# glennhickey/teHmm

Measured on NVIDIA B200. Metric: hmm_trellis_cells_per_sec_fwd_bwd_viterbi, higher is better.
Workload: dtype f32

## Files before the change

### tehmm_b200/csrc/api.cu

```cuda
#include "common.cuh"
#include <algorithm>
#include <cstdarg>
#include <cstdio>
#include <cstring>
#include <string>
#include <vector>

void tehmm_launch_strict_emission(cudaStream_t, const void *, int, int64_t, int, const double *, int, int, double *, double, const double *, unsigned long long *);
void tehmm_launch_strict_forward(cudaStream_t, int64_t, int, const double *, const double *, const double *, const double *, double *);
void tehmm_launch_strict_backward(cudaStream_t, int64_t, int, const double *, const double *, const double *, double *);
void tehmm_launch_strict_viterbi(cudaStream_t, int64_t, int, const double *, const double *, const double *, const double *, int16_t *, int64_t *, double *);
void tehmm_launch_strict_lneta(cudaStream_t, int64_t, int, const double *, const double *, const double *, const double *, double, const double *, double *);
void tehmm_launch_strict_accumulate(cudaStream_t, const void *, int, int64_t, int, double *, int, int, const double *, const double *);
void tehmm_launch_strict_counts(cudaStream_t, const void *, int, int, int64_t, int64_t, int, double *, int, int, const double *);
size_t tehmm_emission_table_budget(int K);
int tehmm_launch_emission(cudaStream_t, const TehmmModelDev &, const TehmmBatchDev &, int, const double *, void *, void *, double *, double *, int *, int, cudaError_t *, int64_t, int64_t);
bool tehmm_emission_rows_ok(const TehmmModelDev &, int, const double *);
cudaError_t tehmm_launch_forward(cudaStream_t, const TehmmModelDev &, const TehmmBatchDev &, int, const void *, const double *, const double *, void *, void *, void *, double *, const int *, int, int);
cudaError_t tehmm_launch_verify(cudaStream_t, const TehmmBatchDev &, int, int, void *, const void *, double, int, int, int *, int *, double *);
cudaError_t tehmm_launch_forward_logprob(cudaStream_t, const TehmmBatchDev &, int, int, const void *, const double *, const double *, double *);
cudaError_t tehmm_launch_backward(cudaStream_t, const TehmmModelDev &, const TehmmBatchDev &, int, int, const void *, const void *, const double *, void *, uint8_t *, double *, void *, void *, void *, void *, void *, const int *, int, int);
cudaError_t tehmm_launch_trans_reduce(cudaStream_t, const TehmmModelDev &, const TehmmBatchDev &, int, const void *, const void *, const void *, double *);
cudaError_t tehmm_launch_map_reduce(cudaStream_t, const TehmmBatchDev &, const double *, double *);
cudaError_t tehmm_launch_viterbi(cudaStream_t, const TehmmModelDev &, const TehmmBatchDev &, int, const void *, const double *, void *, void *, void *, const int *, int, int, const double *, double *);
bool tehmm_viterbi_dp_scores(const TehmmModelDev &, int, const double *);
cudaError_t tehmm_launch_vit_score_reduce(cudaStream_t, const TehmmBatchDev &, const double *, double *);
cudaError_t tehmm_launch_traceback(cudaStream_t, const TehmmModelDev &, const TehmmBatchDev &, int, const void *, const double *, uint8_t *, int64_t *, uint8_t *, uint8_t *, const uint8_t *, const int *, int, int);
cudaError_t tehmm_launch_tb_verify(cudaStream_t, const TehmmBatchDev &, uint8_t *, const uint8_t *, uint8_t *, int *, int *);
cudaError_t tehmm_launch_rescore(cudaStream_t, const TehmmModelDev &, const TehmmBatchDev &, const uint8_t *, const double *, const double *, double *, double *, int64_t, int64_t);
cudaError_t tehmm_launch_emission_stats(cudaStream_t, const TehmmModelDev &, const TehmmBatchDev &, int, const void *, const double *, double *, double *, int, int);
size_t tehmm_stats_smem_bytes(int tab_rows, int N, int K, int prec);
cudaError_t tehmm_launch_widen(cudaStream_t, const uint8_t *, int64_t *, int64_t);
cudaError_t tehmm_launch_forward_tile(cudaStream_t, const TehmmModelDev &, const TehmmBatchDev &, const float *, const double *, float *, float *, float *, double *, const int *, int, int, int64_t);
cudaError_t tehmm_launch_backward_tile(cudaStream_t, const TehmmModelDev &, const TehmmBatchDev &, int, const float *, const float *, float *, uint8_t *, double *, float *, float *, const int *, int, int, int64_t, int);
int tehmm_tile_warps(void);
bool tehmm_forward_umma_ok(const TehmmModelDev &, const TehmmBatchDev &, int, int64_t);
cudaError_t tehmm_launch_forward_umma(cudaStream_t, const TehmmModelDev &, const TehmmBatchDev &, const float *, const double *, float *, float *, float *, double *, int, int64_t, int *, int);
bool tehmm_backward_umma_ok(const TehmmModelDev &, const TehmmBatchDev &, int, int, int64_t);
cudaError_t tehmm_launch_backward_umma(cudaStream_t, const TehmmModelDev &, const TehmmBatchDev &, int, const float *, const float *, float *, uint8_t *, double *, float *, float *, int, int64_t, int *);
cudaError_t tehmm_launch_xi_tile(cudaStream_t, const TehmmModelDev &, const TehmmBatchDev &, const float *, const float *, double *, float *, double *, int);
size_t tehmm_xi_tile_scratch_bytes(int sms);
cudaError_t tehmm_launch_convert(cudaStream_t, int, const void *, double *, int64_t);
cudaError_t tehmm_launch_transfer_ops(cudaStream_t, const TehmmModelDev &, const TehmmChunk *, const int64_t *, int64_t, int, int, const void *, void *, double *, int);
cudaError_t tehmm_launch_ratio_fold(cudaStream_t, const TehmmModelDev &, int64_t, int, const double *, void *, double *, int);
cudaError_t tehmm_launch_ratio_diag(cudaStream_t, const TehmmModelDev &, const TehmmBatchDev &, int, const double *, const void *, double *, double *, int);
cudaError_t tehmm_launch_chain(cudaStream_t, const TehmmModelDev &, int, int, int, const int64_t *, const int64_t *, int64_t, const void *, const double *, const void *, void *);

static thread_local std::string g_err;
static int fail(int code, const char *fmt, ...)
{
    char buf[512];
    va_list ap;
    va_start(ap, fmt);
    vsnprintf(buf, sizeof buf, fmt, ap);
    va_end(ap);
    g_err = buf;
    return code;
}
void tehmm_set_error(int code, const char *msg) { (void)code; g_err = msg ? msg : ""; }
void tehmm_hostpipe_release(tehmm_ctx *c);
#define CU(x)                                                                                 \
    do {                                                                                      \
        cudaError_t e__ = (x);                                                                \
        if (e__ != cudaSuccess)                                                               \
            return fail(TEHMM_ECUDA, "%s failed: %s (%s:%d)", #x, cudaGetErrorString(e__),    \
                        __FILE__, __LINE__);                                                  \
    } while (0)

struct DevBuf {
    void *p = nullptr;
    ~DevBuf() { if (p) cudaFree(p); }
    cudaError_t alloc(size_t n) { return cudaMalloc(&p, n ? n : 1); }
    template <typename T> T *as() { return (T *)p; }
};

#define TEHMM_TRING 32
#define TEHMM_NPENDING 64
enum { TK_EMISSION, TK_FORWARD, TK_BACKWARD, TK_VITERBI_DP, TK_TRACEBACK, TK_RESCORE, TK_STATS, TK_XI, TEHMM_NTIMED };
static const char *const tk_names[TEHMM_NTIMED] = {"us_emission", "us_forward", "us_backward", "us_viterbi_dp",
                                                    "us_traceback", "us_rescore", "us_emission_stats", "us_xi"};

struct tehmm_ctx {
    int device = 0;
    int sms = 148;
    cudaStream_t stream = nullptr;
    cudaStream_t own_stream = nullptr;
    int64_t launches = 0;
    int64_t opt_chunk_tiles = 0, opt_warmup = 0, opt_max_repair = 0;
    int64_t opt_tile = 1, opt_fine_len = 0;
    int64_t opt_timing = 0;
    int64_t opt_umma = 0;
    int64_t opt_umma64 = 1;
    int *d_fault = nullptr;
    int64_t stat_umma_passes = 0;
    int64_t opt_rescore = 0;
    int64_t opt_bwd_tmap = 0;
    int64_t opt_xi_tile = 1;
    int64_t opt_fallback_after = 2;
    int64_t stat_fallbacks = 0, stat_fallback_chunks = 0, stat_noise_accepted = 0;
    double mix_rho = -1.0;
    std::vector<double> mix_A;
    int mix_N = 0;
    cudaEvent_t ev[TEHMM_NTIMED][TEHMM_TRING][2] = {};
    int ev_n[TEHMM_NTIMED] = {};
    int64_t stat_repair_fwd = 0, stat_repair_bwd = 0, stat_repair_vit = 0;
    int64_t stat_tile_passes = 0;
    int64_t stat_bad_fwd = 0, stat_bad_bwd = 0, stat_bad_vit = 0, stat_bad_tb = 0, stat_repair_tb = 0;
    int *h_nbad = nullptr;
    int64_t opt_defer = 0;
    int *h_pending = nullptr;
    int npending = 0;
    int64_t stat_deferred_checks = 0, stat_deferred_bad = 0;
    bool has_model = false;
    TehmmModelDev m{};
    void *model_blob = nullptr;
    size_t model_blob_bytes = 0;
    std::vector<unsigned char> model_key;
    bool has_batch = false;
    TehmmBatchDev b{};
    TehmmBatchDev bf{};
    std::vector<int64_t> batch_key;
    void *batch_blob = nullptr;
    size_t batch_blob_bytes = 0;
    int *d_seq_flag = nullptr;
    int64_t seq_flag_n = 0;
    int64_t max_tiles_per_chunk = 1;
    int64_t fine_len = 0;
};

// ... 56 lines not shown
{
    if (!c) return fail(TEHMM_EINVAL, "ctx is NULL");
    CU(cudaSetDevice(c->device));
    CU(cudaStreamSynchronize(c->stream));
    return TEHMM_OK;
}

int tehmm_ctx_set_stream(tehmm_ctx *c, uint64_t stream)
{
    if (!c) return fail(TEHMM_EINVAL, "ctx is NULL");
    CU(cudaSetDevice(c->device));
    CU(cudaStreamSynchronize(c->stream));
    c->stream = stream == UINT64_MAX ? c->own_stream : (cudaStream_t)(uintptr_t)stream;
    return TEHMM_OK;
}

uint64_t tehmm_ctx_stream(tehmm_ctx *c) { return c ? (uint64_t)(uintptr_t)c->stream : 0; }
int64_t tehmm_ctx_launch_count(tehmm_ctx *c) { return c ? c->launches : 0; }

int tehmm_ctx_set_option(tehmm_ctx *c, const char *name, int64_t v)
{
    if (!c || !name) return fail(TEHMM_EINVAL, "NULL argument");
    if (!strcmp(name, "chunk_tiles")) c->opt_chunk_tiles = v;
    else if (!strcmp(name, "warmup")) c->opt_warmup = v;
    else if (!strcmp(name, "max_repair")) c->opt_max_repair = v;
    else if (!strcmp(name, "tile")) c->opt_tile = v;
    else if (!strcmp(name, "timing")) { c->opt_timing = v; for (int i = 0; i < TEHMM_NTIMED; ++i) c->ev_n[i] = 0; }
    else if (!strcmp(name, "fine_len")) c->opt_fine_len = v;
    else if (!strcmp(name, "umma")) c->opt_umma = v;
    else if (!strcmp(name, "umma64")) c->opt_umma64 = v;
    else if (!strcmp(name, "xi_tile")) c->opt_xi_tile = v;
    else if (!strcmp(name, "defer")) c->opt_defer = v;
    else if (!strcmp(name, "bwd_tmap")) c->opt_bwd_tmap = v;
    else if (!strcmp(name, "rescore")) c->opt_rescore = v;
    else if (!strcmp(name, "fallback_after")) c->opt_fallback_after = v;
    else return fail(TEHMM_EINVAL, "unknown option %s", name);
    return TEHMM_OK;
}

static double mix_rho_of(tehmm_ctx *c)
{
    if (c->mix_rho >= 0.0) return c->mix_rho;
    const int N = c->mix_N;
    if (N <= 0 || c->mix_A.size() != (size_t)N * N) return 0.0;
    const std::vector<double> &A = c->mix_A;
    std::vector<double> pi(N, 1.0 / N), tmp(N), B((size_t)N * N), B2((size_t)N * N);
    for (int it = 0; it < 2000; ++it) {
        double sum = 0.0;
        for (int j = 0; j < N; ++j) tmp[j] = 0.0;
        for (int i = 0; i < N; ++i) {
            const double p = pi[i];
            for (int j = 0; j < N; ++j) tmp[j] += p * A[(size_t)i * N + j];
        }
        for (int j = 0; j < N; ++j) sum += tmp[j];
        for (int j = 0; j < N; ++j) pi[j] = sum > 0.0 ? tmp[j] / sum : 1.0 / N;
    }
    for (int i = 0; i < N; ++i) for (int j = 0; j < N; ++j) B[(size_t)i * N + j] = A[(size_t)i * N + j] - pi[j];
    double lognorm = 0.0;
    for (int sq = 0; sq < 8; ++sq) {
        double f = 0.0;
        for (double v : B) f += v * v;
        f = sqrt(f);
        if (!(f > 0.0)) { lognorm = -INFINITY; break; }
        for (double &v : B) v /= f;
        lognorm = 2.0 * (lognorm + log(f));
        for (int i = 0; i < N; ++i)
// ... 881 lines not shown
                       const double *d_ratios, void *d_post, uint8_t *d_map_states,
                       double *d_map_score, double *d_start_trans, void *d_scratch)
{
    RUN_PROLOGUE();
    if (!d_blin || !d_alpha || !d_scratch) return fail(TEHMM_EINVAL, "NULL argument");
    if ((flags & TEHMM_BWD_POSTERIORS) && !d_post) return fail(TEHMM_EINVAL, "POSTERIORS needs d_post");
    if ((flags & TEHMM_BWD_MAP) && (!d_map_states || !d_map_score)) return fail(TEHMM_EINVAL, "MAP needs d_map_states and d_map_score");
    if ((flags & TEHMM_BWD_TRANS) && !d_start_trans) return fail(TEHMM_EINVAL, "TRANS needs d_start_trans");
    const Scratch s = carve(c, prec);
    char *w = (char *)d_scratch;
    void *sv = w + s.start_vec, *ev = w + s.end_vec;
    double *mp = (double *)(w + s.part_a);
    int *bad = (int *)(w + s.bad), *nbad = (int *)(w + s.nbad);
    void *xi = w + s.xi, *xd = w + s.xdiag, *g0 = w + s.gamma0;
    const int grid = scan_grid(c);
    const bool xi_tile = use_tile(c, prec, d_ratios) && (flags & TEHMM_BWD_TRANS) && (flags & TEHMM_BWD_POSTERIORS) &&
                         !(flags & TEHMM_BWD_RENORM_EPS) && c->opt_xi_tile != 0;
    if (xi_tile) flags &= ~TEHMM_BWD_TRANS;
    const bool tile = use_tile(c, prec, d_ratios) && !(flags & TEHMM_BWD_TRANS);
    const bool wide_umma = c->opt_umma64 != 0 && c->opt_tile != 0 && prec == TEHMM_F32 && c->m.NS == 2 && c->m.LD == 64 &&
                           d_ratios == nullptr && c->b.nseq == 1 && !(flags & TEHMM_BWD_TRANS);
    const TehmmBatchDev &PB = (tile || wide_umma) ? c->bf : c->b;
    bool umma_used = false;
    auto launch = [&](int mode) -> cudaError_t {
        if (wide_umma && tehmm_backward_umma_ok(c->m, PB, flags, mode, c->fine_len)) {
            cudaError_t eu = tehmm_launch_backward_umma(st, c->m, PB, flags, (const float *)d_blin, (const float *)d_alpha, (float *)d_post,
                                                        d_map_states, mp, (float *)sv, (float *)ev, c->sms, c->fine_len, c->d_fault);
            if (eu == cudaSuccess) { c->stat_umma_passes += 1; umma_used = true; return eu; }
            if (eu != cudaErrorNotSupported) return eu;
            cudaGetLastError();
        }
        if (tile) {
            c->stat_tile_passes += 1;
            return tehmm_launch_backward_tile(st, c->m, PB, flags, (const float *)d_blin, (const float *)d_alpha, (float *)d_post, d_map_states, mp, (float *)sv, (float *)ev, bad, mode, c->sms, c->fine_len, (int)c->opt_bwd_tmap);
        }
        return tehmm_launch_backward(st, c->m, PB, prec, flags, d_blin, d_alpha, d_ratios, d_post, d_map_states, mp, xi, xd, g0, sv, ev, bad, mode, grid);
    };
    tk_begin(c, TK_BACKWARD);
    CU(launch(0));
    tk_end(c, TK_BACKWARD);
    c->launches += 1;
    double tol = tolerance(prec, false);
    const int64_t max_pass = c->opt_max_repair > 0 ? c->opt_max_repair : PB.nchunks + 1;
    int fb_rounds = 0;
    for (int64_t pass = 0;; ++pass) {
        CU(tehmm_launch_verify(st, PB, prec, c->m.NP, sv, ev, tol, -1, 1, bad, nbad, nullptr));
        c->launches += 1;
        int nb = 0;
        if (umma_used && pass == 0) CU(cudaMemcpyAsync(c->h_nbad + 1, c->d_fault, sizeof(int), cudaMemcpyDeviceToHost, st));
        if (read_nbad(c, nbad, &nb, !umma_used)) return TEHMM_ECUDA;
        if (umma_used && pass == 0 && c->h_nbad[1]) {
            CU(cudaMemsetAsync(c->d_fault, 0, sizeof(int), st));
            return fail(TEHMM_ECUDA, "bwd_umma_kernel: a barrier wait timed out (tensor-memory protocol fault)");
        }
        if (pass == 0) adapt_warmup(c, nb, PB.nchunks);
        if (nb == 0) break;
        if (pass >= max_pass) return fail(TEHMM_ESTATE, "backward repair did not converge (%d chunks left)", nb);
        if (c->opt_fallback_after >= 0 && pass >= c->opt_fallback_after && d_ratios == nullptr && fb_rounds < TEHMM_MAX_FALLBACK_ROUNDS) {
            if (resolve_flagged(c, st, PB, prec, 1, d_blin, sv, ev, bad, (int64_t)8 << (2 * fb_rounds))) return TEHMM_ECUDA;
            tol = tolerance_after_fallback(c, prec, false);
            fb_rounds += 1;
        }
        c->stat_repair_bwd += 1; c->stat_bad_bwd += nb;
        CU(launch(1));
        c->launches += 1;
    }
    if (flags & TEHMM_BWD_MAP) { CU(tehmm_launch_map_reduce(st, PB, mp, d_map_score)); c->launches += 1; }
// ... 185 lines not shown
```

### tehmm_b200/csrc/tile.cu

```cuda
#include "scan.cuh"
#include <type_traits>
#include <cuda.h>
#include <cstring>

#define TILE_WARPS 8
#ifndef TEHMM_TILE_TENSOR
#define TEHMM_TILE_TENSOR 1
#endif
#ifndef FWD_NBL
#define FWD_NBL 2
#endif
#ifndef FWD_NBS
#define FWD_NBS 1
#endif
#define BWD_STAGES 5
#define TILE_STAGE_BYTES 2048
#define TILE_NEVER 0x7fffffff

struct TransFrag {
    uint32_t hi[4][4][2];
    uint32_t lo[4][4][2];
};

__device__ __forceinline__ uint32_t tf32_rna(float x)
// ... 438 lines not shown
                if (ev) {
#pragma unroll
                    for (int r = 0; r < 2; ++r)
                        if (k + 1 == ke[r]) store_row_vec32(end_vec + cid[r] * 32 + 8 * q, xp, r);
                    kev = next_event(k + 1);
                }
            }
            if (storing) issue_store(j);
        };
        for (int j = 0; j < nblk; ++j) {
            if (kev < kb + (j + 1) * TB) block_step(j, std::true_type());
            else block_step(j, std::false_type());
        }
        nblk_done += (uint32_t)nblk;
        if (alpha) {
            if (lane < 16) bulk_wait<0>();
            __syncwarp();
        }

        for (int rr = 0; rr < 16; ++rr) {
            const int64_t c = gi * 16 + rr;
            if (c >= b.nchunks) break;
            if (mode == 1 && !bad[c]) continue;
            const TehmmChunk ch = b.chunks[c];
            double ms = 0.0;
            for (int64_t tt = ch.t0 + lane; tt < ch.t1; tt += 32) ms += rowmax[tt];
            ms = warp_sum(ms);
            const int e = __shfl_sync(TEHMM_FULL, (rr & 8) ? esum[1] : esum[0], (rr & 7) * 4);
            if (lane == 0) cscale[c] = (double)e * 0.6931471805599453094 + ms;
        }
    }
}

template <int OUT>
__global__ void __launch_bounds__(TILE_WARPS * 32, 1)
bwd_tile_kernel(TehmmModelDev m, TehmmBatchDev b, int flags, const float *__restrict__ blin,
                const float *__restrict__ alpha, float *__restrict__ post,
                uint8_t *__restrict__ map_states, double *__restrict__ map_part,
                float *__restrict__ start_vec, float *__restrict__ end_vec,
                const int *__restrict__ bad, int mode, int64_t group0)
{
    constexpr bool want_post = (OUT & TEHMM_BWD_POSTERIORS) != 0;
    constexpr bool want_map = (OUT & TEHMM_BWD_MAP) != 0;
    extern __shared__ __align__(128) unsigned char tile_smem[];
    const int lane = threadIdx.x & 31, warp = threadIdx.x >> 5;
    const int g = lane >> 2, q = lane & 3;
    const int N = m.N, W = b.warmup;
    constexpr int LD = 32;
    const uint32_t slot0 = (uint32_t)__cvta_generic_to_shared(tile_smem) +
                           (uint32_t)(warp * BWD_STAGES * 2 * TILE_STAGE_BYTES + lane * 16);
    constexpr bool renorm = (OUT & TEHMM_BWD_RENORM_EPS) != 0;
    const float eps32 = 1.1920928955078125e-07f;
    const double renorm_inv = 1.0 / (1.0 + (double)N * 1.1920928955078125e-07);
    const float renorm_invf = (float)renorm_inv;

    TransFrag A;
    load_trans<true>(m, g, q, A);
    float ones[8];
#pragma unroll
    for (int i = 0; i < 8; ++i) ones[i] = 8 * q + i < N ? 1.f : 0.f;

    const int64_t ngroups = (b.nchunks + 15) / 16;
    for (int64_t gi = group0 + (int64_t)blockIdx.x * TILE_WARPS + warp; gi < ngroups;
         gi += (int64_t)gridDim.x * TILE_WARPS) {
        int ks[2], ke[2], kbv[2];
        int64_t off[2], trow[2], cid[2];
        bool exact[2], succ[2];
        int kb = TILE_NEVER, kmax = 0;
#pragma unroll
        for (int r = 0; r < 2; ++r) {
            const int64_t c = gi * 16 + g + 8 * r;
            cid[r] = c;
            bool valid = c < b.nchunks;
            if (valid && mode == 1) valid = bad[c] != 0;
            ks[r] = TILE_NEVER; ke[r] = 0; kbv[r] = TILE_NEVER; off[r] = 0; trow[r] = 0;
            exact[r] = false; succ[r] = false;
            if (valid) {
                const TehmmChunk ch = b.chunks[c];
                const int64_t rem = ch.s1 - ch.t1;
                succ[r] = rem > 0;
                if (rem == 0) { ks[r] = W; exact[r] = true; }
                else if (mode == 1) ks[r] = W;
                else if (rem <= W) { ks[r] = W - (int)rem; exact[r] = true; }
                else ks[r] = 0;
                kbv[r] = exact[r] ? ks[r] + 1 : ks[r];
                ke[r] = W + (int)(ch.t1 - ch.t0);
                trow[r] = ch.t1 - 1 + W;
                off[r] = trow[r] * LD + 8 * q;
                kb = min(kb, ks[r]);
                kmax = max(kmax, ke[r]);
            }
        }
        kb = __reduce_min_sync(TEHMM_FULL, kb);
        kmax = __reduce_max_sync(TEHMM_FULL, kmax);
        if (kmax <= 0) continue;

        auto next_event = [&](int k) -> int {
            int e = TILE_NEVER;
#pragma unroll
            for (int r = 0; r < 2; ++r) {
                if (ks[r] >= k) e = min(e, ks[r]);
                if (ke[r] - 1 >= k) e = min(e, ke[r] - 1);
            }
            return __reduce_min_sync(TEHMM_FULL, e);
        };

        u64 up[8];
        float scp[2] = {1.f, 1.f};
        double mapsum[2] = {0.0, 0.0};
#pragma unroll
        for (int c = 0; c < 8; ++c) up[c] = 0ull;

        const float *lb[2], *la[2];
        float *pp_[2];
        uint8_t *mp_[2];
#pragma unroll
        for (int r = 0; r < 2; ++r) {
            lb[r] = blin + off[r] + LD - (int64_t)kb * LD;
            la[r] = alpha + off[r] - (int64_t)kb * LD;
            pp_[r] = want_post ? post + off[r] - (int64_t)kb * LD : nullptr;
            mp_[r] = want_map ? map_states + trow[r] - kb : nullptr;
        }
        auto issue = [&](int k, int stage) {
#pragma unroll
            for (int r = 0; r < 2; ++r) {
                const uint32_t sl = slot0 + (uint32_t)(stage * 2 * TILE_STAGE_BYTES + r * 1024);
                stage_row(sl, lb[r], k >= kbv[r] && k < ke[r]);
                stage_row(sl + TILE_STAGE_BYTES, la[r], k >= W && k < ke[r]);
                lb[r] -= LD;
                la[r] -= LD;
            }
            stage_commit();
        };

        u64 prq[8];
        bool actq[2] = {false, false}, pend = false;
        auto post_out = [&](const u64 (&pr)[8], const bool (&actr)[2], int back) {
            u64 zs = 0ull;
#pragma unroll
            for (int c = 0; c < 8; ++c) zs = fadd2(zs, pr[c]);
            const float Z0 = quad_sum(lo2(zs)), Z1 = quad_sum(hi2(zs));
            const float invZ[2] = {__frcp_rn(Z0), __frcp_rn(Z1)};
#pragma unroll
            for (int r = 0; r < 2; ++r) {
                const bool act = actr[r];
                float p[8];
#pragma unroll
                for (int c = 0; c < 8; ++c) p[c] = r ? hi2(pr[c]) : lo2(pr[c]);
                if constexpr (want_map) {
                    const float best = quad_max(fmaxf(fmax3(fmax3(p[0], p[1], p[2]), p[3], p[4]), fmax3(p[5], p[6], p[7])));
                    int idx = 99;
#pragma unroll
                    for (int i = 7; i >= 0; --i)
                        if (p[i] == best) idx = 8 * q + i;
                    idx = min(idx, __shfl_xor_sync(TEHMM_FULL, idx, 1));
                    idx = min(idx, __shfl_xor_sync(TEHMM_FULL, idx, 2));
                    const float bg = act ? best * invZ[r] : 0.f;
                    mapsum[r] += renorm ? (act ? ((double)bg + (double)eps32) * renorm_inv : 0.0) : (double)bg;
                    if (act && q == 0) mp_[r][back] = (uint8_t)(idx < N ? idx : 0);
                }
                if constexpr (want_post) {
                    float gv[8];
#pragma unroll
                    for (int i = 0; i < 8; ++i) {
                        gv[i] = p[i] * invZ[r];
                        if (renorm) gv[i] = (gv[i] + eps32) * renorm_invf * ones[i];
                    }
                    store_row8(pp_[r] + (int64_t)back * LD, act, gv);
                }
            }
        };

#pragma unroll
        for (int v = 0; v < BWD_STAGES - 1; ++v) issue(kb + v, v);
        int rs = 0, ws = BWD_STAGES - 1;
        int kev = next_event(kb);
        auto clock_step = [&](const int k, auto evtag) {
            constexpr bool EVC = decltype(evtag)::value;
            issue(k + BWD_STAGES - 1, ws);
            stage_wait<BWD_STAGES - 1>();
            float at[2][8], bt[2][8];
            const uint32_t sl = slot0 + (uint32_t)(rs * 2 * TILE_STAGE_BYTES);
            stage_read(sl, bt[0]);
            stage_read(sl + 1024, bt[1]);
            stage_read(sl + TILE_STAGE_BYTES, at[0]);
            stage_read(sl + TILE_STAGE_BYTES + 1024, at[1]);
            const bool ev = EVC;
            if constexpr (EVC) {
#pragma unroll
                for (int r = 0; r < 2; ++r) {
                    if (k == ks[r] && !exact[r]) {
                        float v[8];
                        if (mode == 1) load_vec32(start_vec + cid[r] * 32 + 8 * q, v);
                        else {
#pragma unroll
                            for (int i = 0; i < 8; ++i) v[i] = ones[i];
                        }
                        set_row(up, r, v);
                        scp[r] = 1.f;
                    }
                }
            }
            u64 wp[8];
            {
                u64 bs[2][4];
#pragma unroll
                for (int r = 0; r < 2; ++r) {
                    const u64 s2 = pk2(scp[r], scp[r]);
#pragma unroll
                    for (int p = 0; p < 4; ++p) bs[r][p] = fmul2(pk2(bt[r][2 * p], bt[r][2 * p + 1]), s2);
                }
#pragma unroll
                for (int p = 0; p < 4; ++p) {
                    wp[2 * p] = pk2(lo2(up[2 * p]) * lo2(bs[0][p]), hi2(up[2 * p]) * lo2(bs[1][p]));
                    wp[2 * p + 1] = pk2(lo2(up[2 * p + 1]) * hi2(bs[0][p]), hi2(up[2 * p + 1]) * hi2(bs[1][p]));
                }
            }
            float acc[4][4];
            tile_matmul(wp, A, acc);
            if (pend) post_out(prq, actq, 1);
            float m0 = 0.f, m1 = 0.f;
#pragma unroll
            for (int nt = 0; nt < 4; ++nt) {
                up[2 * nt] = pk2(acc[nt][0], acc[nt][2]);
                up[2 * nt + 1] = pk2(acc[nt][1], acc[nt][3]);
                m0 = fmax3(m0, acc[nt][0], acc[nt][1]);
                m1 = fmax3(m1, acc[nt][2], acc[nt][3]);
            }
            if constexpr (EVC) {
#pragma unroll
                for (int r = 0; r < 2; ++r) {
                    if (k == ks[r] && exact[r]) {
                        set_row(up, r, ones);
                        if (r == 0) m0 = 1.f; else m1 = 1.f;
                    }
                }
            }
            {
                int dummy;
                scale_of(quad_max(m0), scp[0], dummy);
                scale_of(quad_max(m1), scp[1], dummy);
            }
            if (k >= W) {
#pragma unroll
                for (int c = 0; c < 8; ++c) prq[c] = pk2(lo2(up[c]) * at[0][c], hi2(up[c]) * at[1][c]);
                actq[0] = k < ke[0];
                actq[1] = k < ke[1];
                pend = true;
            } else if (k == W - 1 && mode == 0) {
#pragma unroll
                for (int r = 0; r < 2; ++r)
                    if (succ[r] && k >= ks[r] && k < ke[r]) store_row_vec32(start_vec + cid[r] * 32 + 8 * q, up, r);
            }
            if constexpr (EVC) {
#pragma unroll
                for (int r = 0; r < 2; ++r)
                    if (k + 1 == ke[r]) store_row_vec32(end_vec + cid[r] * 32 + 8 * q, up, r);
                kev = next_event(k + 1);
            }
#pragma unroll
            for (int r = 0; r < 2; ++r) {
                if constexpr (want_post) pp_[r] -= LD;
                if constexpr (want_map) mp_[r] -= 1;
            }
            rs = rs + 1 == BWD_STAGES ? 0 : rs + 1;
            ws = ws + 1 == BWD_STAGES ? 0 : ws + 1;
        };
        for (int k = kb; k < kmax;) {
            clock_step(k, std::true_type());
            ++k;
            const int stop = min(kmax, kev);
            for (; k < stop; ++k) clock_step(k, std::false_type());
        }
        stage_wait<0>();
        if (pend) post_out(prq, actq, 1);
        if constexpr (want_map) {
#pragma unroll
            for (int r = 0; r < 2; ++r)
                if (q == 0 && ke[r] > 0) map_part[cid[r]] = mapsum[r];
        }
    }
}

#define BT_TB 2
#define BT_NB 3
#define BT_BOX (16 * BT_TB * 128)
#define BT_WARP_BYTES (BT_NB * 2 * BT_BOX + 128)

template <int OUT>
__global__ void __launch_bounds__(TILE_WARPS * 32, 1)
bwd_tile_tmap_kernel(TehmmModelDev m, TehmmBatchDev b, int flags, float *__restrict__ post,
                     uint8_t *__restrict__ map_states, double *__restrict__ map_part,
                     float *__restrict__ start_vec, float *__restrict__ end_vec,
                     const __grid_constant__ CUtensorMap tmap_b1, const __grid_constant__ CUtensorMap tmap_a,
                     int lf, int64_t ngroups)
{
    constexpr bool want_post = (OUT & TEHMM_BWD_POSTERIORS) != 0;
    constexpr bool want_map = (OUT & TEHMM_BWD_MAP) != 0;
    extern __shared__ __align__(128) unsigned char tile_smem[];
    const int lane = threadIdx.x & 31, warp = threadIdx.x >> 5;
    const int g = lane >> 2, q = lane & 3;
    const int N = m.N, W = b.warmup;
    constexpr int LD = 32;
    const uint32_t wbase = (uint32_t)__cvta_generic_to_shared(tile_smem) + (uint32_t)(warp * BT_WARP_BYTES);
    const uint32_t bars = wbase + BT_NB * 2 * BT_BOX;
    const uint32_t myoff = (uint32_t)(g * BT_TB * 128 + 32 * q);
    if (lane == 0) {
#pragma unroll
        for (int i = 0; i < BT_NB; ++i) mbar_init(bars + 8 * i, 1);
        asm volatile("fence.mbarrier_init.release.cluster;" ::: "memory");
    }
    fence_async_smem();
// ... 348 lines not shown
                  CU_TENSOR_MAP_INTERLEAVE_NONE, CU_TENSOR_MAP_SWIZZLE_NONE, CU_TENSOR_MAP_L2_PROMOTION_L2_128B,
                  CU_TENSOR_MAP_FLOAT_OOB_FILL_NONE) == CUDA_SUCCESS;
}

cudaError_t tehmm_launch_forward_tile(cudaStream_t st, const TehmmModelDev &m, const TehmmBatchDev &b,
                                      const float *blin, const double *rowmax, float *alpha,
                                      float *start_vec, float *end_vec, double *cscale,
                                      const int *bad, int mode, int sms, int64_t fine_len)
{
    const int smem = TILE_WARPS * FWD_WARP_BYTES;
    cudaError_t e = cudaFuncSetAttribute(fwd_tile_kernel, cudaFuncAttributeMaxDynamicSharedMemorySize, smem);
    if (e != cudaSuccess) return e;
    CUtensorMap tm, tma;
    memset(&tm, 0, sizeof tm);
    memset(&tma, 0, sizeof tma);
    int lf = 0, nfull = 0;
    if (TEHMM_TILE_TENSOR && b.nseq == 1 && fine_len > 0 && mode == 0 &&
        make_lattice_tmap(&tm, blin, fine_len, b.total / fine_len) &&
        (!alpha || make_lattice_tmap(&tma, alpha, fine_len, b.total / fine_len))) {
        lf = (int)fine_len;
        nfull = (int)(b.total / fine_len);
    }
    fwd_tile_kernel<<<tile_grid(b, sms), TILE_WARPS * 32, smem, st>>>(m, b, blin, rowmax, alpha, start_vec,
                                                                      end_vec, cscale, bad, mode, tm, tma, lf, nfull);
    return cudaGetLastError();
}

static bool make_lattice_tmap_tb(CUtensorMap *tm, const float *base, int64_t lf, int64_t nfull, int tb);

cudaError_t tehmm_launch_backward_tile(cudaStream_t st, const TehmmModelDev &m, const TehmmBatchDev &b,
                                       int flags, const float *blin, const float *alpha, float *post,
                                       uint8_t *map_states, double *map_part, float *start_vec,
                                       float *end_vec, const int *bad, int mode, int sms, int64_t fine_len,
                                       int use_tmap)
{
    const int th = TILE_WARPS * 32;
    const int smem = TILE_WARPS * BWD_STAGES * 2 * TILE_STAGE_BYTES;
    const int out = flags & (TEHMM_BWD_POSTERIORS | TEHMM_BWD_MAP);
    const int outr = flags & (TEHMM_BWD_POSTERIORS | TEHMM_BWD_MAP | TEHMM_BWD_RENORM_EPS);
    int64_t group0 = 0;
    if (TEHMM_TILE_TENSOR && use_tmap && b.nseq == 1 && mode == 0 && fine_len > b.warmup && fine_len % BT_TB == 0 &&
        b.warmup % BT_TB == 0 && b.warmup >= BT_TB) {
        const int64_t lf = fine_len;
        const int64_t nfull_b = std::min<int64_t>(b.total / lf, (b.total - 1) / lf);
        const int64_t ngroups = nfull_b > 0 ? (nfull_b - 1) / 16 : 0;
        CUtensorMap tmb, tma;
        memset(&tmb, 0, sizeof tmb);
        memset(&tma, 0, sizeof tma);
        if (ngroups > 0 && make_lattice_tmap_tb(&tmb, blin + 32, lf, nfull_b, BT_TB) &&
            make_lattice_tmap_tb(&tma, alpha, lf, nfull_b, BT_TB)) {
            const int tsmem = TILE_WARPS * BT_WARP_BYTES;
            const int64_t need = (ngroups + TILE_WARPS - 1) / TILE_WARPS;
            const int tgrid = (int)(need < sms ? need : sms);
#define BWD_TMAP(O) do { cudaError_t e = cudaFuncSetAttribute(bwd_tile_tmap_kernel<O>, cudaFuncAttributeMaxDynamicSharedMemorySize, tsmem); \
                         if (e != cudaSuccess) return e; \
                         bwd_tile_tmap_kernel<O><<<tgrid, th, tsmem, st>>>(m, b, flags, post, map_states, map_part, start_vec, end_vec, tmb, tma, (int)lf, ngroups); } while (0)
            switch (out) {
            case 0: BWD_TMAP(0); break;
            case TEHMM_BWD_POSTERIORS: BWD_TMAP(TEHMM_BWD_POSTERIORS); break;
            case TEHMM_BWD_MAP: BWD_TMAP(TEHMM_BWD_MAP); break;
            default: BWD_TMAP(TEHMM_BWD_POSTERIORS | TEHMM_BWD_MAP); break;
            }
#undef BWD_TMAP
            cudaError_t e = cudaGetLastError();
            if (e != cudaSuccess) return e;
            group0 = ngroups;
        }
    }
    const int64_t left = (b.nchunks + 15) / 16 - group0;
    if (left <= 0) return cudaSuccess;
    const int64_t need = (left + TILE_WARPS - 1) / TILE_WARPS;
    const int grid = (int)(need < 1 ? 1 : (need < sms ? need : sms));
#define BWD_TILE(O) do { cudaError_t e = cudaFuncSetAttribute(bwd_tile_kernel<O>, cudaFuncAttributeMaxDynamicSharedMemorySize, smem); \
                         if (e != cudaSuccess) return e; \
                         bwd_tile_kernel<O><<<grid, th, smem, st>>>(m, b, flags, blin, alpha, post, map_states, map_part, start_vec, end_vec, bad, mode, group0); } while (0)
    switch (outr) {
    case 0: BWD_TILE(0); break;
    case TEHMM_BWD_POSTERIORS: BWD_TILE(TEHMM_BWD_POSTERIORS); break;
    case TEHMM_BWD_MAP: BWD_TILE(TEHMM_BWD_MAP); break;
    case TEHMM_BWD_POSTERIORS | TEHMM_BWD_MAP: BWD_TILE(TEHMM_BWD_POSTERIORS | TEHMM_BWD_MAP); break;
    case TEHMM_BWD_RENORM_EPS: BWD_TILE(0); break;
    case TEHMM_BWD_POSTERIORS | TEHMM_BWD_RENORM_EPS: BWD_TILE(TEHMM_BWD_POSTERIORS | TEHMM_BWD_RENORM_EPS); break;
    case TEHMM_BWD_MAP | TEHMM_BWD_RENORM_EPS: BWD_TILE(TEHMM_BWD_MAP | TEHMM_BWD_RENORM_EPS); break;
    default: BWD_TILE(TEHMM_BWD_POSTERIORS | TEHMM_BWD_MAP | TEHMM_BWD_RENORM_EPS); break;
    }
#undef BWD_TILE
    return cudaGetLastError();
}

int tehmm_tile_warps(void) { return TILE_WARPS; }

cudaError_t tehmm_launch_xi_tile(cudaStream_t st, const TehmmModelDev &m, const TehmmBatchDev &b,
                                 const float *alpha, const float *post, double *xi_part, float *gamma0,
                                 double *start_trans, int sms)
{
    const int smem = TILE_WARPS * 2 * 16 * XI_LDS * 4;
    const int64_t need = (b.nchunks + TILE_WARPS - 1) / TILE_WARPS;
    const int grid = (int)(need < 1 ? 1 : (need < sms ? need : sms));
    cudaError_t e = cudaFuncSetAttribute(xi_tile_kernel, cudaFuncAttributeMaxDynamicSharedMemorySize, smem);
    if (e != cudaSuccess) return e;
    xi_tile_kernel<<<grid, TILE_WARPS * 32, smem, st>>>(m, b, alpha, post, xi_part, gamma0);
    xi_reduce_kernel<<<(m.N * m.N + 127) / 128, 128, 0, st>>>(m, b, xi_part, grid * TILE_WARPS, gamma0, start_trans);
    return cudaGetLastError();
}
size_t tehmm_xi_tile_scratch_bytes(int sms) { return (size_t)sms * TILE_WARPS * 1024 * sizeof(double); }
```

Measured before the change: 97.62 billion.

## Split backward tile kernel into recurrence and epilogue warp groups

Adds a warp-specialized variant of the backward tile kernel. Recurrence warps publish beta rows through an mbarrier-guarded shared-memory ring. A second group of epilogue warps loads alpha, forms the posteriors and MAP states, and writes the outputs. Registers are redistributed with setmaxnreg, and the beta stage read is moved after the matmul so it can overlap. This is meant to take the posterior/MAP output work off the serial recurrence critical path, at the cost of twice the threads, extra shared memory and barrier handshakes.

```diff
diff --git a/tehmm_b200/csrc/api.cu b/tehmm_b200/csrc/api.cu
--- a/tehmm_b200/csrc/api.cu
+++ b/tehmm_b200/csrc/api.cu
@@ -32,7 +32,7 @@
 size_t tehmm_stats_smem_bytes(int tab_rows, int N, int K, int prec);
 cudaError_t tehmm_launch_widen(cudaStream_t, const uint8_t *, int64_t *, int64_t);
 cudaError_t tehmm_launch_forward_tile(cudaStream_t, const TehmmModelDev &, const TehmmBatchDev &, const float *, const double *, float *, float *, float *, double *, const int *, int, int, int64_t);
-cudaError_t tehmm_launch_backward_tile(cudaStream_t, const TehmmModelDev &, const TehmmBatchDev &, int, const float *, const float *, float *, uint8_t *, double *, float *, float *, const int *, int, int, int64_t, int);
+cudaError_t tehmm_launch_backward_tile(cudaStream_t, const TehmmModelDev &, const TehmmBatchDev &, int, const float *, const float *, float *, uint8_t *, double *, float *, float *, const int *, int, int, int64_t, int, int);
 int tehmm_tile_warps(void);
 bool tehmm_forward_umma_ok(const TehmmModelDev &, const TehmmBatchDev &, int, int64_t);
 cudaError_t tehmm_launch_forward_umma(cudaStream_t, const TehmmModelDev &, const TehmmBatchDev &, const float *, const double *, float *, float *, float *, double *, int, int64_t, int *, int);
@@ -95,6 +95,7 @@
     int64_t stat_umma_passes = 0;
     int64_t opt_rescore = 0;
     int64_t opt_bwd_tmap = 0;
+    int64_t opt_bwd_split = 1;
     int64_t opt_xi_tile = 1;
     int64_t opt_fallback_after = 2;
     int64_t stat_fallbacks = 0, stat_fallback_chunks = 0, stat_noise_accepted = 0;
@@ -217,6 +218,7 @@
     else if (!strcmp(name, "xi_tile")) c->opt_xi_tile = v;
     else if (!strcmp(name, "defer")) c->opt_defer = v;
     else if (!strcmp(name, "bwd_tmap")) c->opt_bwd_tmap = v;
+    else if (!strcmp(name, "bwd_split")) c->opt_bwd_split = v;
     else if (!strcmp(name, "rescore")) c->opt_rescore = v;
     else if (!strcmp(name, "fallback_after")) c->opt_fallback_after = v;
     else return fail(TEHMM_EINVAL, "unknown option %s", name);
@@ -1164,7 +1166,7 @@
         }
         if (tile) {
             c->stat_tile_passes += 1;
-            return tehmm_launch_backward_tile(st, c->m, PB, flags, (const float *)d_blin, (const float *)d_alpha, (float *)d_post, d_map_states, mp, (float *)sv, (float *)ev, bad, mode, c->sms, c->fine_len, (int)c->opt_bwd_tmap);
+            return tehmm_launch_backward_tile(st, c->m, PB, flags, (const float *)d_blin, (const float *)d_alpha, (float *)d_post, d_map_states, mp, (float *)sv, (float *)ev, bad, mode, c->sms, c->fine_len, (int)c->opt_bwd_tmap, (int)c->opt_bwd_split);
         }
         return tehmm_launch_backward(st, c->m, PB, prec, flags, d_blin, d_alpha, d_ratios, d_post, d_map_states, mp, xi, xd, g0, sv, ev, bad, mode, grid);
     };
diff --git a/tehmm_b200/csrc/tile.cu b/tehmm_b200/csrc/tile.cu
--- a/tehmm_b200/csrc/tile.cu
+++ b/tehmm_b200/csrc/tile.cu
@@ -494,8 +494,111 @@
     }
 }
 
+struct BwdRows {
+    int ks[2], ke[2], kbv[2];
+    int64_t off[2], trow[2], cid[2];
+    bool exact[2], succ[2];
+    int kb, kmax;
+};
+__device__ __forceinline__ void bwd_rows(const TehmmBatchDev &b, int64_t gi, int g, int q, int W,
+                                         const int *__restrict__ bad, int mode, BwdRows &s)
+{
+    constexpr int LD = 32;
+    s.kb = TILE_NEVER;
+    s.kmax = 0;
+#pragma unroll
+    for (int r = 0; r < 2; ++r) {
+        const int64_t c = gi * 16 + g + 8 * r;
+        s.cid[r] = c;
+        bool valid = c < b.nchunks;
+        if (valid && mode == 1) valid = bad[c] != 0;
+        s.ks[r] = TILE_NEVER; s.ke[r] = 0; s.kbv[r] = TILE_NEVER; s.off[r] = 0; s.trow[r] = 0;
+        s.exact[r] = false; s.succ[r] = false;
+        if (valid) {
+            const TehmmChunk ch = b.chunks[c];
+            const int64_t rem = ch.s1 - ch.t1;
+            s.succ[r] = rem > 0;
+            if (rem == 0) { s.ks[r] = W; s.exact[r] = true; }
+            else if (mode == 1) s.ks[r] = W;
+            else if (rem <= W) { s.ks[r] = W - (int)rem; s.exact[r] = true; }
+            else s.ks[r] = 0;
+            s.kbv[r] = s.exact[r] ? s.ks[r] + 1 : s.ks[r];
+            s.ke[r] = W + (int)(ch.t1 - ch.t0);
+            s.trow[r] = ch.t1 - 1 + W;
+            s.off[r] = s.trow[r] * LD + 8 * q;
+            s.kb = min(s.kb, s.ks[r]);
+            s.kmax = max(s.kmax, s.ke[r]);
+        }
+    }
+    s.kb = __reduce_min_sync(TEHMM_FULL, s.kb);
+    s.kmax = __reduce_max_sync(TEHMM_FULL, s.kmax);
+}
+
 template <int OUT>
-__global__ void __launch_bounds__(TILE_WARPS * 32, 1)
+__device__ __forceinline__ void bwd_post_out(const u64 (&pr)[8], const bool (&actr)[2], int back, int q, int N,
+                                             const float (&ones)[8], double renorm_inv, float renorm_invf,
+                                             double (&mapsum)[2], float *const (&pp_)[2], uint8_t *const (&mp_)[2])
+{
+    constexpr bool want_post = (OUT & TEHMM_BWD_POSTERIORS) != 0;
+    constexpr bool want_map = (OUT & TEHMM_BWD_MAP) != 0;
+    constexpr bool renorm = (OUT & TEHMM_BWD_RENORM_EPS) != 0;
+    constexpr int LD = 32;
+    const float eps32 = 1.1920928955078125e-07f;
+    u64 zs = 0ull;
+#pragma unroll
+    for (int c = 0; c < 8; ++c) zs = fadd2(zs, pr[c]);
+    const float Z0 = quad_sum(lo2(zs)), Z1 = quad_sum(hi2(zs));
+    const float invZ[2] = {__frcp_rn(Z0), __frcp_rn(Z1)};
+#pragma unroll
+    for (int r = 0; r < 2; ++r) {
+        const bool act = actr[r];
+        float p[8];
+#pragma unroll
+        for (int c = 0; c < 8; ++c) p[c] = r ? hi2(pr[c]) : lo2(pr[c]);
+        if constexpr (want_map) {
+            const float best = quad_max(fmaxf(fmax3(fmax3(p[0], p[1], p[2]), p[3], p[4]), fmax3(p[5], p[6], p[7])));
+            int idx = 99;
+#pragma unroll
+            for (int i = 7; i >= 0; --i)
+                if (p[i] == best) idx = 8 * q + i;
+            idx = min(idx, __shfl_xor_sync(TEHMM_FULL, idx, 1));
+            idx = min(idx, __shfl_xor_sync(TEHMM_FULL, idx, 2));
+            const float bg = act ? best * invZ[r] : 0.f;
+            mapsum[r] += renorm ? (act ? ((double)bg + (double)eps32) * renorm_inv : 0.0) : (double)bg;
+            if (act && q == 0) mp_[r][back] = (uint8_t)(idx < N ? idx : 0);
+        }
+        if constexpr (want_post) {
+            float gv[8];
+#pragma unroll
+            for (int i = 0; i < 8; ++i) {
+                gv[i] = p[i] * invZ[r];
+                if (renorm) gv[i] = (gv[i] + eps32) * renorm_invf * ones[i];
+            }
+            store_row8(pp_[r] + (int64_t)back * LD, act, gv);
+        }
+    }
+}
+
+__device__ __forceinline__ void mbar_arrive(uint32_t bar)
+{
+    asm volatile("mbarrier.arrive.shared::cta.b64 _, [%0];" :: "r"(bar) : "memory");
+}
+__device__ __forceinline__ void sts_u64x2(uint32_t a, u64 x, u64 y)
+{
+    asm volatile("st.shared.v2.u64 [%0], {%1,%2};" :: "r"(a), "l"(x), "l"(y) : "memory");
+}
+__device__ __forceinline__ void lds_u64x2(uint32_t a, u64 &x, u64 &y)
+{
+    asm volatile("ld.shared.v2.u64 {%0,%1}, [%2];" : "=l"(x), "=l"(y) : "r"(a) : "memory");
+}
+
+#define BWD_RING 3
+#define BWD_REC_REGS 168
+#define BWD_EPI_REGS 88
+#define BWD_SPLIT_SMEM (TILE_WARPS * (BWD_RING * TILE_STAGE_BYTES + 2 * BWD_RING * 8))
+
+template <int OUT, bool SPLIT>
+__global__ void __launch_bounds__((SPLIT ? 2 : 1) * TILE_WARPS * 32, 1)
 bwd_tile_kernel(TehmmModelDev m, TehmmBatchDev b, int flags, const float *__restrict__ blin,
                 const float *__restrict__ alpha, float *__restrict__ post,
                 uint8_t *__restrict__ map_states, double *__restrict__ map_part,
@@ -505,64 +608,121 @@
     constexpr bool want_post = (OUT & TEHMM_BWD_POSTERIORS) != 0;
     constexpr bool want_map = (OUT & TEHMM_BWD_MAP) != 0;
     extern __shared__ __align__(128) unsigned char tile_smem[];
-    const int lane = threadIdx.x & 31, warp = threadIdx.x >> 5;
+    const int lane = threadIdx.x & 31, warp = (threadIdx.x >> 5) % TILE_WARPS;
     const int g = lane >> 2, q = lane & 3;
     const int N = m.N, W = b.warmup;
     constexpr int LD = 32;
-    const uint32_t slot0 = (uint32_t)__cvta_generic_to_shared(tile_smem) +
-                           (uint32_t)(warp * BWD_STAGES * 2 * TILE_STAGE_BYTES + lane * 16);
-    constexpr bool renorm = (OUT & TEHMM_BWD_RENORM_EPS) != 0;
-    const float eps32 = 1.1920928955078125e-07f;
+    const uint32_t smem0 = (uint32_t)__cvta_generic_to_shared(tile_smem);
+    const uint32_t slot0 = smem0 + (uint32_t)(warp * BWD_STAGES * 2 * TILE_STAGE_BYTES + lane * 16);
+    const uint32_t ring0 = smem0 + (uint32_t)(TILE_WARPS * BWD_STAGES * 2 * TILE_STAGE_BYTES +
+                                              warp * BWD_RING * TILE_STAGE_BYTES + lane * 16);
+    const uint32_t full0 = smem0 + (uint32_t)(TILE_WARPS * (BWD_STAGES * 2 + BWD_RING) * TILE_STAGE_BYTES +
+                                              warp * 2 * BWD_RING * 8);
+    const uint32_t empty0 = full0 + BWD_RING * 8;
     const double renorm_inv = 1.0 / (1.0 + (double)N * 1.1920928955078125e-07);
     const float renorm_invf = (float)renorm_inv;
+    float ones[8];
+#pragma unroll
+    for (int i = 0; i < 8; ++i) ones[i] = 8 * q + i < N ? 1.f : 0.f;
+    const int64_t ngroups = (b.nchunks + 15) / 16;
+
+    if constexpr (SPLIT) {
+        if (threadIdx.x < TILE_WARPS * 32 && lane == 0) {
+#pragma unroll
+            for (int i = 0; i < BWD_RING; ++i) {
+                mbar_init(full0 + 8 * i, 32);
+                mbar_init(empty0 + 8 * i, 32);
+            }
+            asm volatile("fence.mbarrier_init.release.cluster;" ::: "memory");
+        }
+        __syncthreads();
+        if (threadIdx.x >= TILE_WARPS * 32) {
+            asm volatile("setmaxnreg.dec.sync.aligned.u32 %0;" :: "n"(BWD_EPI_REGS));
+            uint32_t n = 0;
+            for (int64_t gi = group0 + (int64_t)blockIdx.x * TILE_WARPS + warp; gi < ngroups;
+                 gi += (int64_t)gridDim.x * TILE_WARPS) {
+                BwdRows s;
+                bwd_rows(b, gi, g, q, W, bad, mode, s);
+                if (s.kmax <= 0) continue;
+                double mapsum[2] = {0.0, 0.0};
+                const float *la[2];
+                float *pp_[2];
+                uint8_t *mp_[2];
+#pragma unroll
+                for (int r = 0; r < 2; ++r) {
+                    la[r] = alpha + s.off[r] - (int64_t)W * LD;
+                    pp_[r] = want_post ? post + s.off[r] - (int64_t)W * LD : nullptr;
+                    mp_[r] = want_map ? map_states + s.trow[r] - W : nullptr;
+                }
+                auto issue = [&](int k, int stage) {
+#pragma unroll
+                    for (int r = 0; r < 2; ++r) {
+                        stage_row(slot0 + (uint32_t)(stage * 2 * TILE_STAGE_BYTES + TILE_STAGE_BYTES + r * 1024),
+                                  la[r], k < s.ke[r]);
+                        la[r] -= LD;
+                    }
+                    stage_commit();
+                };
+#pragma unroll
+                for (int v = 0; v < BWD_STAGES - 1; ++v) issue(W + v, v);
+                int rs = 0, ws = BWD_STAGES - 1;
+                for (int k = W; k < s.kmax; ++k) {
+                    issue(k + BWD_STAGES - 1, ws);
+                    stage_wait<BWD_STAGES - 1>();
+                    float at[2][8];
+                    const uint32_t sl = slot0 + (uint32_t)(rs * 2 * TILE_STAGE_BYTES + TILE_STAGE_BYTES);
+                    stage_read(sl, at[0]);
+                    stage_read(sl + 1024, at[1]);
+                    const uint32_t slot = n % BWD_RING;
+                    mbar_wait(full0 + 8 * slot, (n / BWD_RING) & 1u);
+                    u64 up[8];
+#pragma unroll
+                    for (int i = 0; i < 4; ++i)
+                        lds_u64x2(ring0 + slot * TILE_STAGE_BYTES + (uint32_t)(i * 512), up[2 * i], up[2 * i + 1]);
+                    mbar_arrive(empty0 + 8 * slot);
+                    ++n;
+                    u64 pr[8];
+#pragma unroll
+                    for (int c = 0; c < 8; ++c) pr[c] = pk2(lo2(up[c]) * at[0][c], hi2(up[c]) * at[1][c]);
+                    const bool act[2] = {k < s.ke[0], k < s.ke[1]};
+                    bwd_post_out<OUT>(pr, act, 0, q, N, ones, renorm_inv, renorm_invf, mapsum, pp_, mp_);
+#pragma unroll
+                    for (int r = 0; r < 2; ++r) {
+                        if constexpr (want_post) pp_[r] -= LD;
+                        if constexpr (want_map) mp_[r] -= 1;
+                    }
+                    rs = rs + 1 == BWD_STAGES ? 0 : rs + 1;
+                    ws = ws + 1 == BWD_STAGES ? 0 : ws + 1;
+                }
+                stage_wait<0>();
+                if constexpr (want_map) {
+#pragma unroll
+                    for (int r = 0; r < 2; ++r)
+                        if (q == 0 && s.ke[r] > 0) map_part[s.cid[r]] = mapsum[r];
+                }
+            }
+            return;
+        }
+        asm volatile("setmaxnreg.inc.sync.aligned.u32 %0;" :: "n"(BWD_REC_REGS));
+    }
 
     TransFrag A;
     load_trans<true>(m, g, q, A);
-    float ones[8];
-#pragma unroll
-    for (int i = 0; i < 8; ++i) ones[i] = 8 * q + i < N ? 1.f : 0.f;
-
-    const int64_t ngroups = (b.nchunks + 15) / 16;
+    uint32_t npub = 0;
+
     for (int64_t gi = group0 + (int64_t)blockIdx.x * TILE_WARPS + warp; gi < ngroups;
          gi += (int64_t)gridDim.x * TILE_WARPS) {
-        int ks[2], ke[2], kbv[2];
-        int64_t off[2], trow[2], cid[2];
-        bool exact[2], succ[2];
-        int kb = TILE_NEVER, kmax = 0;
-#pragma unroll
-        for (int r = 0; r < 2; ++r) {
-            const int64_t c = gi * 16 + g + 8 * r;
-            cid[r] = c;
-            bool valid = c < b.nchunks;
-            if (valid && mode == 1) valid = bad[c] != 0;
-            ks[r] = TILE_NEVER; ke[r] = 0; kbv[r] = TILE_NEVER; off[r] = 0; trow[r] = 0;
-            exact[r] = false; succ[r] = false;
-            if (valid) {
-                const TehmmChunk ch = b.chunks[c];
-                const int64_t rem = ch.s1 - ch.t1;
-                succ[r] = rem > 0;
-                if (rem == 0) { ks[r] = W; exact[r] = true; }
-                else if (mode == 1) ks[r] = W;
-                else if (rem <= W) { ks[r] = W - (int)rem; exact[r] = true; }
-                else ks[r] = 0;
-                kbv[r] = exact[r] ? ks[r] + 1 : ks[r];
-                ke[r] = W + (int)(ch.t1 - ch.t0);
-                trow[r] = ch.t1 - 1 + W;
-                off[r] = trow[r] * LD + 8 * q;
-                kb = min(kb, ks[r]);
-                kmax = max(kmax, ke[r]);
-            }
-        }
-        kb = __reduce_min_sync(TEHMM_FULL, kb);
-        kmax = __reduce_max_sync(TEHMM_FULL, kmax);
+        BwdRows s;
+        bwd_rows(b, gi, g, q, W, bad, mode, s);
+        const int kb = s.kb, kmax = s.kmax;
         if (kmax <= 0) continue;
 
         auto next_event = [&](int k) -> int {
             int e = TILE_NEVER;
 #pragma unroll
             for (int r = 0; r < 2; ++r) {
-                if (ks[r] >= k) e = min(e, ks[r]);
-                if (ke[r] - 1 >= k) e = min(e, ke[r] - 1);
+                if (s.ks[r] >= k) e = min(e, s.ks[r]);
+                if (s.ke[r] - 1 >= k) e = min(e, s.ke[r] - 1);
             }
             return __reduce_min_sync(TEHMM_FULL, e);
         };
@@ -578,82 +738,52 @@
         uint8_t *mp_[2];
 #pragma unroll
         for (int r = 0; r < 2; ++r) {
-            lb[r] = blin + off[r] + LD - (int64_t)kb * LD;
-            la[r] = alpha + off[r] - (int64_t)kb * LD;
-            pp_[r] = want_post ? post + off[r] - (int64_t)kb * LD : nullptr;
-            mp_[r] = want_map ? map_states + trow[r] - kb : nullptr;
+            lb[r] = blin + s.off[r] + LD - (int64_t)kb * LD;
+            la[r] = alpha + s.off[r] - (int64_t)kb * LD;
+            pp_[r] = want_post ? post + s.off[r] - (int64_t)kb * LD : nullptr;
+            mp_[r] = want_map ? map_states + s.trow[r] - kb : nullptr;
         }
         auto issue = [&](int k, int stage) {
 #pragma unroll
             for (int r = 0; r < 2; ++r) {
                 const uint32_t sl = slot0 + (uint32_t)(stage * 2 * TILE_STAGE_BYTES + r * 1024);
-                stage_row(sl, lb[r], k >= kbv[r] && k < ke[r]);
-                stage_row(sl + TILE_STAGE_BYTES, la[r], k >= W && k < ke[r]);
+                stage_row(sl, lb[r], k >= s.kbv[r] && k < s.ke[r]);
                 lb[r] -= LD;
-                la[r] -= LD;
+                if constexpr (!SPLIT) {
+                    stage_row(sl + TILE_STAGE_BYTES, la[r], k >= W && k < s.ke[r]);
+                    la[r] -= LD;
+                }
             }
             stage_commit();
         };
 
         u64 prq[8];
         bool actq[2] = {false, false}, pend = false;
-        auto post_out = [&](const u64 (&pr)[8], const bool (&actr)[2], int back) {
-            u64 zs = 0ull;
-#pragma unroll
-            for (int c = 0; c < 8; ++c) zs = fadd2(zs, pr[c]);
-            const float Z0 = quad_sum(lo2(zs)), Z1 = quad_sum(hi2(zs));
-            const float invZ[2] = {__frcp_rn(Z0), __frcp_rn(Z1)};
-#pragma unroll
-            for (int r = 0; r < 2; ++r) {
-                const bool act = actr[r];
-                float p[8];
-#pragma unroll
-                for (int c = 0; c < 8; ++c) p[c] = r ? hi2(pr[c]) : lo2(pr[c]);
-                if constexpr (want_map) {
-                    const float best = quad_max(fmaxf(fmax3(fmax3(p[0], p[1], p[2]), p[3], p[4]), fmax3(p[5], p[6], p[7])));
-                    int idx = 99;
-#pragma unroll
-                    for (int i = 7; i >= 0; --i)
-                        if (p[i] == best) idx = 8 * q + i;
-                    idx = min(idx, __shfl_xor_sync(TEHMM_FULL, idx, 1));
-                    idx = min(idx, __shfl_xor_sync(TEHMM_FULL, idx, 2));
-                    const float bg = act ? best * invZ[r] : 0.f;
-                    mapsum[r] += renorm ? (act ? ((double)bg + (double)eps32) * renorm_inv : 0.0) : (double)bg;
-                    if (act && q == 0) mp_[r][back] = (uint8_t)(idx < N ? idx : 0);
-                }
-                if constexpr (want_post) {
-                    float gv[8];
-#pragma unroll
-                    for (int i = 0; i < 8; ++i) {
-                        gv[i] = p[i] * invZ[r];
-                        if (renorm) gv[i] = (gv[i] + eps32) * renorm_invf * ones[i];
-                    }
-                    store_row8(pp_[r] + (int64_t)back * LD, act, gv);
-                }
-            }
-        };
 
 #pragma unroll
         for (int v = 0; v < BWD_STAGES - 1; ++v) issue(kb + v, v);
         int rs = 0, ws = BWD_STAGES - 1;
         int kev = next_event(kb);
+        float bt[2][8];
+        stage_wait<BWD_STAGES - 2>();
+        stage_read(slot0, bt[0]);
+        stage_read(slot0 + 1024, bt[1]);
         auto clock_step = [&](const int k, auto evtag) {
             constexpr bool EVC = decltype(evtag)::value;
             issue(k + BWD_STAGES - 1, ws);
-            stage_wait<BWD_STAGES - 1>();
-            float at[2][8], bt[2][8];
-            const uint32_t sl = slot0 + (uint32_t)(rs * 2 * TILE_STAGE_BYTES);
-            stage_read(sl, bt[0]);
-            stage_read(sl + 1024, bt[1]);
-            stage_read(sl + TILE_STAGE_BYTES, at[0]);
-            stage_read(sl + TILE_STAGE_BYTES + 1024, at[1]);
-            const bool ev = EVC;
+            float at[2][8];
+            (void)at;
+            if constexpr (!SPLIT) {
+                const uint32_t sl = slot0 + (uint32_t)(rs * 2 * TILE_STAGE_BYTES);
+                stage_read(sl + TILE_STAGE_BYTES, at[0]);
+                stage_read(sl + TILE_STAGE_BYTES + 1024, at[1]);
+            }
             if constexpr (EVC) {
 #pragma unroll
                 for (int r = 0; r < 2; ++r) {
-                    if (k == ks[r] && !exact[r]) {
+                    if (k == s.ks[r] && !s.exact[r]) {
                         float v[8];
-                        if (mode == 1) load_vec32(start_vec + cid[r] * 32 + 8 * q, v);
+                        if (mode == 1) load_vec32(start_vec + s.cid[r] * 32 + 8 * q, v);
                         else {
 #pragma unroll
                             for (int i = 0; i < 8; ++i) v[i] = ones[i];
@@ -680,7 +810,18 @@
             }
             float acc[4][4];
             tile_matmul(wp, A, acc);
-            if (pend) post_out(prq, actq, 1);
+            {
+                stage_wait<BWD_STAGES - 2>();
+                const uint32_t sn = slot0 + (uint32_t)((rs + 1 == BWD_STAGES ? 0 : rs + 1) * 2 * TILE_STAGE_BYTES);
+                stage_read(sn, bt[0]);
+                stage_read(sn + 1024, bt[1]);
+            }
+            if constexpr (SPLIT) {
+                if (k >= W) mbar_wait(empty0 + 8 * (npub % BWD_RING), ((npub / BWD_RING) & 1u) ^ 1u);
+            }
+            if constexpr (!SPLIT) {
+                if (pend) bwd_post_out<OUT>(prq, actq, 1, q, N, ones, renorm_inv, renorm_invf, mapsum, pp_, mp_);
+            }
             float m0 = 0.f, m1 = 0.f;
 #pragma unroll
             for (int nt = 0; nt < 4; ++nt) {
@@ -692,7 +833,7 @@
             if constexpr (EVC) {
 #pragma unroll
                 for (int r = 0; r < 2; ++r) {
-                    if (k == ks[r] && exact[r]) {
+                    if (k == s.ks[r] && s.exact[r]) {
                         set_row(up, r, ones);
                         if (r == 0) m0 = 1.f; else m1 = 1.f;
                     }
@@ -704,26 +845,37 @@
                 scale_of(quad_max(m1), scp[1], dummy);
             }
             if (k >= W) {
-#pragma unroll
-                for (int c = 0; c < 8; ++c) prq[c] = pk2(lo2(up[c]) * at[0][c], hi2(up[c]) * at[1][c]);
-                actq[0] = k < ke[0];
-                actq[1] = k < ke[1];
-                pend = true;
+                if constexpr (SPLIT) {
+                    const uint32_t slot = npub % BWD_RING;
+#pragma unroll
+                    for (int i = 0; i < 4; ++i)
+                        sts_u64x2(ring0 + slot * TILE_STAGE_BYTES + (uint32_t)(i * 512), up[2 * i], up[2 * i + 1]);
+                    mbar_arrive(full0 + 8 * slot);
+                    ++npub;
+                } else {
+#pragma unroll
+                    for (int c = 0; c < 8; ++c) prq[c] = pk2(lo2(up[c]) * at[0][c], hi2(up[c]) * at[1][c]);
+                    actq[0] = k < s.ke[0];
+                    actq[1] = k < s.ke[1];
+                    pend = true;
+                }
             } else if (k == W - 1 && mode == 0) {
 #pragma unroll
                 for (int r = 0; r < 2; ++r)
-                    if (succ[r] && k >= ks[r] && k < ke[r]) store_row_vec32(start_vec + cid[r] * 32 + 8 * q, up, r);
+                    if (s.succ[r] && k >= s.ks[r] && k < s.ke[r]) store_row_vec32(start_vec + s.cid[r] * 32 + 8 * q, up, r);
             }
             if constexpr (EVC) {
 #pragma unroll
                 for (int r = 0; r < 2; ++r)
-                    if (k + 1 == ke[r]) store_row_vec32(end_vec + cid[r] * 32 + 8 * q, up, r);
+                    if (k + 1 == s.ke[r]) store_row_vec32(end_vec + s.cid[r] * 32 + 8 * q, up, r);
                 kev = next_event(k + 1);
             }
-#pragma unroll
-            for (int r = 0; r < 2; ++r) {
-                if constexpr (want_post) pp_[r] -= LD;
-                if constexpr (want_map) mp_[r] -= 1;
+            if constexpr (!SPLIT) {
+#pragma unroll
+                for (int r = 0; r < 2; ++r) {
+                    if constexpr (want_post) pp_[r] -= LD;
+                    if constexpr (want_map) mp_[r] -= 1;
+                }
             }
             rs = rs + 1 == BWD_STAGES ? 0 : rs + 1;
             ws = ws + 1 == BWD_STAGES ? 0 : ws + 1;
@@ -735,11 +887,13 @@
             for (; k < stop; ++k) clock_step(k, std::false_type());
         }
         stage_wait<0>();
-        if (pend) post_out(prq, actq, 1);
-        if constexpr (want_map) {
-#pragma unroll
-            for (int r = 0; r < 2; ++r)
-                if (q == 0 && ke[r] > 0) map_part[cid[r]] = mapsum[r];
+        if constexpr (!SPLIT) {
+            if (pend) bwd_post_out<OUT>(prq, actq, 1, q, N, ones, renorm_inv, renorm_invf, mapsum, pp_, mp_);
+            if constexpr (want_map) {
+#pragma unroll
+                for (int r = 0; r < 2; ++r)
+                    if (q == 0 && s.ke[r] > 0) map_part[s.cid[r]] = mapsum[r];
+            }
         }
     }
 }
@@ -1154,7 +1308,7 @@
                                        int flags, const float *blin, const float *alpha, float *post,
                                        uint8_t *map_states, double *map_part, float *start_vec,
                                        float *end_vec, const int *bad, int mode, int sms, int64_t fine_len,
-                                       int use_tmap)
+                                       int use_tmap, int bwd_split)
 {
     const int th = TILE_WARPS * 32;
     const int smem = TILE_WARPS * BWD_STAGES * 2 * TILE_STAGE_BYTES;
@@ -1193,19 +1347,23 @@
     if (left <= 0) return cudaSuccess;
     const int64_t need = (left + TILE_WARPS - 1) / TILE_WARPS;
     const int grid = (int)(need < 1 ? 1 : (need < sms ? need : sms));
-#define BWD_TILE(O) do { cudaError_t e = cudaFuncSetAttribute(bwd_tile_kernel<O>, cudaFuncAttributeMaxDynamicSharedMemorySize, smem); \
-                         if (e != cudaSuccess) return e; \
-                         bwd_tile_kernel<O><<<grid, th, smem, st>>>(m, b, flags, blin, alpha, post, map_states, map_part, start_vec, end_vec, bad, mode, group0); } while (0)
+    const bool split = bwd_split != 0 && out != 0;
+    const int sth = (split ? 2 : 1) * TILE_WARPS * 32, ssmem = smem + (split ? BWD_SPLIT_SMEM : 0);
+#define BWD_TILE(O, S) do { cudaError_t e = cudaFuncSetAttribute(bwd_tile_kernel<O, S>, cudaFuncAttributeMaxDynamicSharedMemorySize, ssmem); \
+                            if (e != cudaSuccess) return e; \
+                            bwd_tile_kernel<O, S><<<grid, sth, ssmem, st>>>(m, b, flags, blin, alpha, post, map_states, map_part, start_vec, end_vec, bad, mode, group0); } while (0)
+#define BWD_TILE2(O) do { if (split) BWD_TILE(O, true); else BWD_TILE(O, false); } while (0)
     switch (outr) {
-    case 0: BWD_TILE(0); break;
-    case TEHMM_BWD_POSTERIORS: BWD_TILE(TEHMM_BWD_POSTERIORS); break;
-    case TEHMM_BWD_MAP: BWD_TILE(TEHMM_BWD_MAP); break;
-    case TEHMM_BWD_POSTERIORS | TEHMM_BWD_MAP: BWD_TILE(TEHMM_BWD_POSTERIORS | TEHMM_BWD_MAP); break;
-    case TEHMM_BWD_RENORM_EPS: BWD_TILE(0); break;
-    case TEHMM_BWD_POSTERIORS | TEHMM_BWD_RENORM_EPS: BWD_TILE(TEHMM_BWD_POSTERIORS | TEHMM_BWD_RENORM_EPS); break;
-    case TEHMM_BWD_MAP | TEHMM_BWD_RENORM_EPS: BWD_TILE(TEHMM_BWD_MAP | TEHMM_BWD_RENORM_EPS); break;
-    default: BWD_TILE(TEHMM_BWD_POSTERIORS | TEHMM_BWD_MAP | TEHMM_BWD_RENORM_EPS); break;
-    }
+    case 0: BWD_TILE(0, false); break;
+    case TEHMM_BWD_POSTERIORS: BWD_TILE2(TEHMM_BWD_POSTERIORS); break;
+    case TEHMM_BWD_MAP: BWD_TILE2(TEHMM_BWD_MAP); break;
+    case TEHMM_BWD_POSTERIORS | TEHMM_BWD_MAP: BWD_TILE2(TEHMM_BWD_POSTERIORS | TEHMM_BWD_MAP); break;
+    case TEHMM_BWD_RENORM_EPS: BWD_TILE(0, false); break;
+    case TEHMM_BWD_POSTERIORS | TEHMM_BWD_RENORM_EPS: BWD_TILE2(TEHMM_BWD_POSTERIORS | TEHMM_BWD_RENORM_EPS); break;
+    case TEHMM_BWD_MAP | TEHMM_BWD_RENORM_EPS: BWD_TILE2(TEHMM_BWD_MAP | TEHMM_BWD_RENORM_EPS); break;
+    default: BWD_TILE2(TEHMM_BWD_POSTERIORS | TEHMM_BWD_MAP | TEHMM_BWD_RENORM_EPS); break;
+    }
+#undef BWD_TILE2
 #undef BWD_TILE
     return cudaGetLastError();
 }
```

Result: no change. 97.95 billion, median of 6 (+0.3%).
